# Xiaoming-Zhao/PointNav-VO

Measured on AMD Instinct MI355X. Metric: RGB-D frame-pair VO inferences/s @341x192, higher is better.
Workload: dtype f32

## Files before the change

### pointnav-vo_amd/csrc/pnvo_api.hip

```cpp
#include <hip/hip_runtime.h>

#include <cmath>
#include <cstdio>
#include <cstdlib>
#include <cstring>
#include <functional>
#include <atomic>
#include <condition_variable>
#include <map>
#include <mutex>
#include <string>
#include <thread>
#include <vector>

#include "pnvo_model.h"

using namespace pnvo;

thread_local std::string g_err;

int pnvo_fail(pnvo_handle h, int code, const std::string &msg) {
  if (h) h->err = msg;
  g_err = msg;
  return code;
}

long long pnvo_device_bytes_live(void) { return g_device_bytes_live.load(); }

namespace {

inline int fail(pnvo_handle h, int code, const std::string &msg) { return pnvo_fail(h, code, msg); }


Layer make_layer(const std::string &name, const std::string &gn, int cin, int cout, int k, int stride, int pad,
                 int hin, int win, int groups) {
  Layer l;
  l.name = name;
  l.gn = gn;
  l.cin = cin;
  l.cinp = rup(cin, 8);
  l.cout = cout;
  l.coutp = rup(cout, 32);
  l.k = l.kw = k;
  l.stride = stride;
  l.pad = pad;
  l.hin = hin;
  l.win = win;
  l.hout = (hin + 2 * pad - k) / stride + 1;
  l.wout = (win + 2 * pad - k) / stride + 1;
  l.groups = groups;
  return l;
}

void build_plan(pnvo_model_s *m) {
  const pnvo_config &c = m->cfg;
  m->C = c.n_rgb + c.n_depth + c.n_dd + c.n_tdv;
  m->CP = rup(m->C, 8);
  m->CPL = rup(m->C, 16);
  m->Hs = halve(c.height);
  m->Ws = halve(c.width);
  m->Hp = halve(m->Hs);
  m->Wp = halve(m->Ws);
  {
    const int n[4] = {c.n_rgb, c.n_depth, c.n_dd, c.n_tdv};
    int prev_off[4], half = 0;
    for (int t = 0; t < 4; ++t) {
      prev_off[t] = half;
// ... 128 lines not shown
              if (co < cout && ci < cin)
                out[((((size_t)ntg * T + tap) * J + j) * 64 + hh * 32 + n) * 4 + t] =
                    oihw[((size_t)co * cin + ci) * T + tap];
            }
}

namespace {
inline void pack_conv_weight_cinp(const float *oihw, int cout, int cin, int cinp, int kh, int kw, std::vector<float> &out) {
  pnvo_pack_conv_weight_cinp(oihw, cout, cin, cinp, kh, kw, out);
}

int load_conv(pnvo_handle h, const Toc &t, Layer &l, bool has_gn) {
  int rc = PNVO_OK;
  const float *w = find_tensor(h, t, l.name + ".weight", {l.cout, l.cin / l.cgroups, l.k, l.kw}, &rc);
  if (!w) return rc;
  if (l.cgroups > 1) {
    const int cg = l.cin / l.cgroups;
    if (l.cin != l.cout || !conv_group_supported(l.cout, cg, l.k, l.stride, l.pad))
      return fail(h, PNVO_ERR_ARG, "grouped conv " + l.name + ": unsupported geometry (" + std::to_string(l.cout) + " channels in groups of " +
                                       std::to_string(cg) + ")");
    std::vector<float> pk(conv_group_packed_floats(l.cout, cg));
    pack_conv_group_weight(w, l.cout, cg, pk.data());
    HIPCHK(h, l.wpk_grp.upload(pk.data(), pk.size()));
  } else {
    std::vector<float> pk;
    pack_conv_weight_cinp(w, l.cout, l.cin, l.cinp, l.k, l.kw, pk);
    HIPCHK(h, l.wpk.upload(pk.data(), pk.size()));
    l.host_w.assign(w, w + (size_t)l.cout * l.cin * l.k * l.kw);
  }
  if (has_gn) {
    const float *g = find_tensor(h, t, l.gn + ".weight", {l.cout}, &rc);
    if (!g) return rc;
    const float *b = find_tensor(h, t, l.gn + ".bias", {l.cout}, &rc);
    if (!b) return rc;
    HIPCHK(h, l.gamma.upload(g, l.cout));
    HIPCHK(h, l.beta.upload(b, l.cout));
  }
  return PNVO_OK;
}

int reset_contract_flag(pnvo_handle h) {
  if (!h->dd_flag) HIPCHK(h, h->dd_flag.alloc_host(1, hipHostMallocMapped | hipHostMallocCoherent));
  if (!h->dd_flag_dev) HIPCHK(h, h->dd_flag_dev.alloc(1));
  *(volatile int *)h->dd_flag = 0;
  HIPCHK(h, hipMemset(h->dd_flag_dev, 0, sizeof(int)));
  return PNVO_OK;
}

void free_workspace(pnvo_model_s *m) {
  pnvo_drop_graphs(m);
  for (DevBuf<float> *b : {&m->xin, &m->stem_raw, &m->out_ws, &m->bufY[0], &m->bufY[1], &m->rawA, &m->rawB, &m->rawD, &m->rawC, &m->comp_raw,
                           &m->hid, &m->stats, &m->stats_ds, &m->tapbuf})
    b->reset();
  for (DevPair<float> *q : {&m->ssA, &m->ssB, &m->ssD, &m->ssC, &m->ssE}) q->reset();
  m->cap = 0;
}

bool x3_layer(pnvo_handle m, const Layer &l) {
  const bool s2 = l.stride == 2 && m->opt.x3_s2;
  const bool k3 = l.k == 3 && l.kw == 3 && l.pad == 1 && (l.stride == 1 || s2);
  const bool k1 = l.k == 1 && l.kw == 1 && l.pad == 0 && s2;
  return (k3 || k1) && l.cgroups == 1 && !l.host_w.empty() && m->opt.conv <= 1;
}
bool x3_two_pieces(pnvo_handle m, const Layer &l) {
  if (m->bottleneck || !(l.in_bound < 6.0e4f)) return false;
  if (m->train != nullptr)
    return m->opt.train_pieces == 2 && pnvo_train_x2_scale(m, l.name + ".weight") != nullptr;
  return m->opt.pieces == 2;
}
void conv_geometry(const Layer &l, int B, int y_cstride, ConvArgs &a) {
  std::memset(&a, 0, sizeof(a));
  a.B = B;
  a.H = l.hin;
  a.W = l.win;
  a.CIN = l.cinp;
  a.Ho = l.hout;
  a.Wo = l.wout;
  a.COUT = l.cout;
  a.COUTP = l.coutp;
  a.KH = l.k;
  a.KW = l.kw;
  a.stride = l.stride;
  a.pad = l.pad;
  a.y_cstride = y_cstride;
  a.up = 1;
}

double conv_flops(const Layer &l, int B) { return 2.0 * ((double)((long)B * l.hout * l.wout) * l.cout * (l.cin / l.cgroups) * l.k * l.kw); }
double conv_bytes(const Layer &l, int B) {
  return 4.0 * ((double)B * l.hin * l.win * l.cin + (double)((long)B * l.hout * l.wout) * l.cout + (double)l.cout * l.cin * l.k * l.kw);
}

bool ride_fits(pnvo_handle m, const Layer &c1, const Layer &cd) {
  if (!m->opt.ds_fuse || m->tap_dst != nullptr || m->bottleneck || cd.k != 1 || cd.kw != 1 || cd.stride != 2 || cd.pad != 0) return false;
  if (c1.cinp != cd.cinp || c1.coutp != cd.coutp || c1.cout != cd.cout || c1.hout != cd.hout || c1.wout != cd.wout || c1.hin != cd.hin ||
      c1.win != cd.win || c1.cout != c1.coutp || c1.groups != cd.groups || cd.host_w.empty())
    return false;
  return x3_layer(m, cd) && x3_two_pieces(m, cd);
}
}

ConvChoice pnvo_conv_choice(pnvo_handle m, const Layer &l, int B, const ConvAsk &ask) {
  ConvChoice c;
  const int P = l.hout * l.wout;
  c.flops = conv_flops(l, B);
  if (l.cgroups > 1) {
// ... 28 lines not shown
  c.family = lds ? ConvChoice::FP32_LDS : ConvChoice::FP32_GENERIC;
  c.slots = lds ? conv3_lds_slots(a) : conv_slots(P, c.MT);
  return c;
}

bool pnvo_conv_takes_tail(pnvo_handle m, const Layer &l, int B) {
  return m->tap_dst == nullptr && m->opt.tail && pnvo_conv_choice(m, l, B, {}).family == ConvChoice::X3;
}

namespace {
size_t stats_floats(pnvo_handle m, const Layer &l, int B) {
  const PnvoOptions saved = m->opt;
  int slots = 0;
  m->opt.x3_s2 = 1;
  for (m->opt.conv = 1; m->opt.conv <= 3; ++m->opt.conv) slots = std::max(slots, pnvo_conv_choice(m, l, B, {}).slots);
  m->opt = saved;
  return (size_t)B * (size_t)slots * l.coutp * 2;
}

int stem_slots(pnvo_handle m, StemPlan::Kernel k) {
  if (k == StemPlan::GENERIC) return 0;
  if (k == StemPlan::LDS) return stem_tiles_x(m->Ws) * stem_tiles_y(m->Hs);
  return k == StemPlan::MX ? stem_mx_slots(m->Hs, m->Ws) : stem_dd_slots(m->Hs, m->Ws);
}

int ensure_workspace(pnvo_handle m, int B) {
  if (B <= m->cap) return PNVO_OK;
  free_workspace(m);
  const pnvo_config &c = m->cfg;
  const size_t npix = (size_t)B * c.height * c.width;
  size_t act = (size_t)B * m->Hp * m->Wp * c.baseplanes;
  for (size_t k = 1; k < m->convs.size(); ++k) {
    const size_t need = (size_t)B * m->convs[k].hout * m->convs[k].wout * m->convs[k].coutp;
    if (need > act) act = need;
  }
  int maxc = m->comp_cp;
  size_t st = 0;
  for (StemPlan::Kernel k : {StemPlan::MX, StemPlan::DD, StemPlan::LDS}) st = std::max(st, (size_t)B * stem_slots(m, k) * m->convs[0].coutp * 2);
  for (const Layer &l : m->convs) {
    if (l.coutp > maxc) maxc = l.coutp;
    const size_t s = stats_floats(m, l, B);
    if (s > st) st = s;
  }
  (void)npix;
  HIPCHK(m, m->stem_raw.alloc((size_t)B * m->Hs * m->Ws * c.baseplanes));
  HIPCHK(m, m->bufY[0].alloc(act));
  HIPCHK(m, m->bufY[1].alloc(act));
  HIPCHK(m, m->rawA.alloc(act));
  HIPCHK(m, m->rawB.alloc(act));
  HIPCHK(m, m->rawD.alloc(act));
  if (m->bottleneck) HIPCHK(m, m->rawC.alloc(act));
  HIPCHK(m, m->comp_raw.alloc((size_t)B * m->fh * m->fw * m->comp_cp));
  HIPCHK(m, m->hid.alloc((size_t)B * c.hidden));
  HIPCHK(m, m->out_ws.alloc((size_t)B * c.out_dim));
  HIPCHK(m, m->stats.alloc(st));
  HIPCHK(m, m->stats_ds.alloc(st));
  for (int k = 0; k < 2; ++k) {
    HIPCHK(m, m->ssA.alloc(k, (size_t)B * maxc));
    HIPCHK(m, m->ssB.alloc(k, (size_t)B * maxc));
    HIPCHK(m, m->ssD.alloc(k, (size_t)B * maxc));
    if (m->cfg.se) HIPCHK(m, m->ssE.alloc(k, (size_t)B * maxc));
    HIPCHK(m, m->ssC.alloc(k, (size_t)B * m->comp_cp));
    HIPCHK(m, hipMemset(m->ssC[k], 0, (size_t)B * m->comp_cp * sizeof(float)));
  }
  HIPCHK(m, m->tapbuf.alloc((size_t)B * m->fh * m->fw * m->comp_cp));
  HIPCHK(m, m->kpart.reserve((size_t)32 * B * (size_t)std::max(c.hidden, 32)));
  m->cap = B;
  return PNVO_OK;
}

}

PnvoTimed::PnvoTimed(pnvo_model_s *m_, hipStream_t s_, const std::string &name, double flops, double bytes) : m(m_), s(s_) {
  if (!m->timing) return;
  auto it = m->tindex.find(name);
  int idx;
  if (it == m->tindex.end()) {
    pnvo_kernel_time e;
    std::memset(&e, 0, sizeof(e));
    std::snprintf(e.name, sizeof(e.name), "%s", name.c_str());
    idx = (int)m->tentries.size();
    m->tentries.push_back(e);
    m->tindex[name] = idx;
  } else {
    idx = it->second;
  }
  m->tentries[idx].launches += 1;
  m->tentries[idx].flops += flops;
  m->tentries[idx].bytes += bytes;
  TimingRec r;
  auto get = [&]() {
    hipEvent_t e;
    if (!m->evpool.empty()) {
      e = m->evpool.back();
      m->evpool.pop_back();
    } else {
      (void)hipEventCreate(&e);
    }
    return e;
  };
  r.a = get();
  r.b = get();
  r.entry = idx;
  (void)hipEventRecord(r.a, s);
  m->trecs.push_back(r);
  rec = (int)m->trecs.size() - 1;
// ... 512 lines not shown
  GnGroup sgg{0x7fffffff, 0x7fffffff, {nullptr, nullptr}, {nullptr, nullptr}};
  switch (p.kernel) {
    case StemPlan::MX: rc = stem_launch_mx(m, B, r, p, sgg); break;
    case StemPlan::DD: rc = stem_launch_dd(m, B, r, p); break;
    case StemPlan::LDS: {
      StemArgs a;
      stem_lds_args(m, B, r, p.slots, a);
      a.dbg = m->opt.stem_dbg;
      a.lds_pad = m->opt.stem_dbg_pad;
      Timed t = stem_timed(m, B, r, false);
      HIPCHK(m, launch_stem_lds(a, stem.coutp, r.s));
      break;
    }
    case StemPlan::GENERIC:
      return pnvo_run_conv(m, stem, B, {.in_scale = m->stem_sc, .in_shift = m->stem_sh, .y = r.y, .y_cstride = stem.coutp, .ss = r.ss,
                                        .mu = r.mu, .rstd = r.rstd, .src = r.src, .grp = r.grp, .s = r.s});
  }
  if (rc != PNVO_OK) return rc;
  if (p.kernel != StemPlan::LDS) {
    if (p.repairs && (rc = pnvo_stem_standin(m, B, r, p.slots, m->dd_flag_dev)) != PNVO_OK) return rc;
    if ((rc = pnvo_mark_stem(m, r.s, p)) != PNVO_OK) return rc;
  }
  if (r.slots_out != nullptr) *r.slots_out = p.slots;
  return r.skip_finalize ? PNVO_OK : finalize_gn(m, stem, B, p.slots, 0, r.ss, r.mu, r.rstd, r.s, r.grp ? &sgg : nullptr);
}

int pnvo_ensure_workspace(pnvo_handle m, int B) { return ensure_workspace(m, B); }

namespace {
struct OptChoice {
  const char *word;
  int value;
};
struct OptDef {
  const char *key, *env;
  int PnvoOptions::*field;
  bool numeric;
  OptChoice choices[7];
};
const OptDef kOptions[] = {
    {"stem", "PNVO_STEM", &PnvoOptions::stem, false, {{"auto", 0}, {"mx", 1}, {"dd", 2}, {"dense", 3}, {nullptr, 0}}},
    {"conv", "PNVO_CONV", &PnvoOptions::conv, false, {{"auto", 0}, {"x3", 1}, {"fp32", 2}, {"generic", 3}, {nullptr, 0}}},
    {"pieces", "PNVO_PIECES", &PnvoOptions::pieces, false, {{"2", 2}, {"3", 3}, {nullptr, 0}}},
    {"stem_form", "PNVO_STEM_FORM", &PnvoOptions::stem_form, false, {{"auto", 0}, {"tiles", 2}, {"resident", 3}, {"fast", 4}, {nullptr, 0}}},
    {"train_pieces", "PNVO_TRAIN_PIECES", &PnvoOptions::train_pieces, false, {{"2", 2}, {"3", 3}, {nullptr, 0}}},
    {"x3_persist", "PNVO_X3_PERSIST", &PnvoOptions::x3_persist, false, {{"on", 1}, {"off", 0}, {nullptr, 0}}},
    {"x3_rows", "PNVO_X3_ROWS", &PnvoOptions::x3_rows, false, {{"on", 1}, {"off", 0}, {nullptr, 0}}},
    {"x3_strip", "PNVO_X3_STRIP", &PnvoOptions::x3_strip, false, {{"on", 1}, {"off", 0}, {nullptr, 0}}},
    {"x3_fine", "PNVO_X3_FINE", &PnvoOptions::x3_fine, false, {{"on", 1}, {"off", 0}, {nullptr, 0}}},
    {"x3_w8", "PNVO_X3_W8", &PnvoOptions::x3_w8, false, {{"on", 1}, {"off", 0}, {nullptr, 0}}},
    {"x3_m16", "PNVO_X3_M16", &PnvoOptions::x3_m16, false, {{"on", 1}, {"off", 0}, {nullptr, 0}}},
    {"x3_ksplit", "PNVO_X3_KSPLIT", &PnvoOptions::x3_ksplit, false, {{"on", 1}, {"off", 0}, {nullptr, 0}}},
    {"fc_rows", "PNVO_FC_ROWS", &PnvoOptions::fc_rows, true, {{nullptr, 0}}},
    {"head_fuse", "PNVO_HEAD_FUSE", &PnvoOptions::head_fuse, false, {{"on", 1}, {"off", 0}, {nullptr, 0}}},
    {"ds_fuse", "PNVO_DS_FUSE", &PnvoOptions::ds_fuse, false, {{"on", 1}, {"off", 0}, {nullptr, 0}}},
    {"gn_fuse", "PNVO_GN_FUSE", &PnvoOptions::gn_fuse, false, {{"on", 1}, {"off", 0}, {nullptr, 0}}},
    {"x3_s2", nullptr, &PnvoOptions::x3_s2, false, {{"on", 1}, {"off", 0}, {nullptr, 0}}},
    {"tail", "PNVO_TAIL", &PnvoOptions::tail, false, {{"fused", 1}, {"separate", 0}, {nullptr, 0}}},
    {"pool", "PNVO_POOL", &PnvoOptions::pool, false, {{"fused", 1}, {"separate", 0}, {nullptr, 0}}},
    {"graph", "PNVO_GRAPH", &PnvoOptions::graph, true, {{nullptr, 0}}},
    {"stem_dbg", nullptr, &PnvoOptions::stem_dbg, true, {{nullptr, 0}}},
    {"stem_dbg_pad", nullptr, &PnvoOptions::stem_dbg_pad, true, {{nullptr, 0}}},
    {"wgrad_stem", "PNVO_WGRAD_STEM", &PnvoOptions::wgrad_stem, false, {{"mx", 0}, {"fp32", 1}, {nullptr, 0}}},
    {"wgrad3", "PNVO_WGRAD3", &PnvoOptions::wgrad3, false, {{"x3", 1}, {"fp32", 0}, {nullptr, 0}}},
    {"pool_bwd", "PNVO_POOL_BWD", &PnvoOptions::pool_bwd, false, {{"fused", 1}, {"separate", 0}, {nullptr, 0}}},
    {"dgrad", "PNVO_DGRAD", &PnvoOptions::dgrad, false, {{"phase", 1}, {"masked", 0}, {nullptr, 0}}},
    {"bf16_fuse", nullptr, &PnvoOptions::bf16_fuse, false, {{"on", 1}, {"off", 0}, {nullptr, 0}}},
    {"input_fallback", "PNVO_INPUT_FALLBACK", &PnvoOptions::input_fallback, false, {{"on", 1}, {"off", 0}, {nullptr, 0}}},
    {"small_net", "PNVO_SMALL_NET", &PnvoOptions::small_net, false, {{"on", 1}, {"off", 0}, {nullptr, 0}}},
    {"small_max", "PNVO_SMALL_MAX", &PnvoOptions::small_max, true, {{nullptr, 0}}},
    {"small_coop", "PNVO_SMALL_COOP", &PnvoOptions::small_coop, true, {{nullptr, 0}}},
    {"small_prof", "PNVO_SMALL_PROF", &PnvoOptions::small_prof, true, {{nullptr, 0}}},
};

const OptDef *find_option(const char *key) {
  for (const OptDef &d : kOptions)
    if (std::strcmp(d.key, key) == 0) return &d;
  return nullptr;
}

bool parse_option(const OptDef &d, const char *word, int *out) {
  if (d.numeric) {
    char *end = nullptr;
    const long v = std::strtol(word, &end, 10);
    if (end == word || *end != 0) return false;
    *out = (int)v;
    return true;
  }
  for (const OptChoice *c = d.choices; c->word != nullptr; ++c)
    if (std::strcmp(c->word, word) == 0) {
      *out = c->value;
      return true;
    }
  return false;
}

void env_defaults(pnvo_model_s *m) {
  for (const OptDef &d : kOptions) {
    const char *e = d.env ? std::getenv(d.env) : nullptr;
    int v;
    if (e && parse_option(d, e, &v)) m->opt.*(d.field) = v;
  }
  if (std::getenv("PNVO_X3_S2_OFF")) m->opt.x3_s2 = 0;
  if (std::getenv("PNVO_BF16_NOFUSE")) m->opt.bf16_fuse = 0;
  if (const char *e = std::getenv("PNVO_STEM_DBG")) std::sscanf(e, "%d,%d", &m->opt.stem_dbg, &m->opt.stem_dbg_pad);
}
// ... 245 lines not shown
            double ind = 0.0;
            for (int k = 0; k < 30; ++k) {
              const int r = ref[k];
              if (r < 0) continue;
              const double wv = (double)w[((size_t)o * st.cin + r) * T + tap];
              const double sd = (double)h->stdev[r], mu = (double)h->mean[r];
              const double div = slot_tensor[k] == 0 ? 255.0 : 1.0;
              wk[((size_t)o * 32 + k) * T + tap] = (float)(wv / (div * sd));
              ind -= wv * mu / sd;
            }
            wk[((size_t)o * 32 + 30) * T + tap] = (float)ind;
          }
      };
      fold(slot_ref, h->mx_wk);
      fold(slot_ref_sw, h->mx_wk_swapped);
      h->mx_slot_ref = slot_ref;
      h->mx_slot_new = slot_new;
      std::vector<unsigned short> pk(stem_mx_packed_u16(3, st.cout / 32));
      pack_stem_mx_weight(h->mx_wk.data(), st.cout, 3, h->mx_xslot, pk.data());
      HIPCHK(h, h->mx_wpk3.upload(pk.data(), pk.size()));
      {
        std::vector<unsigned short> pk2(stem_mx_packed_u16(2, st.cout / 32));
        h->mx_oscale = pack_stem_mx_weight_h(h->mx_wk.data(), st.cout, h->mx_xslot, pk2.data());
        h->mx_wpk2_dev = false;
        HIPCHK(h, h->mx_wpk2.upload(pk2.data(), pk2.size()));
      }
      {
        std::vector<float> pages(64, 0.f);
        HIPCHK(h, h->mx_pages.upload(pages.data(), pages.size()));
      }
      if ((rc = reset_contract_flag(h)) != PNVO_OK) return rc;
      h->mx_ok = true;
    }
  }
  const int flat = h->comp_c * h->fh * h->fw;
  const int fc_in = flat + (c.act_embed ? 32 : 0);
  const float *w1 = find_tensor(h, t, h->fc.name + ".weight", {c.hidden, fc_in}, &rc);
  if (!w1) return rc;
  const float *b1 = find_tensor(h, t, h->fc.name + ".bias", {c.hidden}, &rc);
  if (!b1) return rc;
  {
    std::vector<float> vis((size_t)c.hidden * flat);
    for (int o = 0; o < c.hidden; ++o) std::memcpy(&vis[(size_t)o * flat], w1 + (size_t)o * fc_in, sizeof(float) * flat);
    std::vector<float> pk;
    h->fc.host_w = vis;
    {
      const int hw = h->fh * h->fw, kp = hw * h->comp_cp;
      std::vector<float> rows((size_t)c.hidden * kp, 0.f);
      for (int o = 0; o < c.hidden; ++o)
        for (int ch = 0; ch < h->comp_c; ++ch)
          for (int q = 0; q < hw; ++q) rows[(size_t)o * kp + (size_t)q * h->comp_cp + ch] = vis[(size_t)o * flat + (size_t)ch * hw + q];
      HIPCHK(h, h->fc_rows_w.upload(rows.data(), rows.size()));
    }
    pack_conv_weight_cinp(vis.data(), c.hidden, h->comp_c, h->comp_cp, h->fh, h->fw, pk);
    HIPCHK(h, h->fc.wpk.upload(pk.data(), pk.size()));
    const int rows = c.act_embed ? c.n_acts + 1 : 1;
    std::vector<float> bias((size_t)rows * c.hidden);
    const float *emb = nullptr;
    if (c.act_embed) {
      emb = find_tensor(h, t, "action_embedding.weight", {c.n_acts + 1, 32}, &rc);
      if (!emb) return rc;
    }
    for (int a = 0; a < rows; ++a)
      for (int o = 0; o < c.hidden; ++o) {
        double acc = 0.0;
        if (emb)
          for (int e = 0; e < 32; ++e) acc += (double)w1[(size_t)o * fc_in + flat + e] * (double)emb[a * 32 + e];
        bias[(size_t)a * c.hidden + o] = (float)(acc + (double)b1[o]);
      }
    HIPCHK(h, h->fc_bias.upload(bias.data(), bias.size()));
  }
  const float *w2 = find_tensor(h, t, "output_head.1.weight", {c.out_dim, c.hidden}, &rc);
  if (!w2) return rc;
  const float *b2 = find_tensor(h, t, "output_head.1.bias", {c.out_dim}, &rc);
  if (!b2) return rc;
  {
    std::vector<float> pk;
    h->head.host_w.assign(w2, w2 + (size_t)c.out_dim * c.hidden);
    pack_conv_weight_cinp(w2, c.out_dim, c.hidden, c.hidden, 1, 1, pk);
    HIPCHK(h, h->head.wpk.upload(pk.data(), pk.size()));
    HIPCHK(h, h->head_bias.upload(b2, c.out_dim));
    HIPCHK(h, h->head_w_plain.upload(w2, (size_t)c.out_dim * c.hidden));
  }
  h->loaded = true;
  h->load_gen += 1;
  h->weights_gen += 1;
  h->weights_gen_at_load = h->weights_gen;
  return PNVO_OK;
}

int pnvo_set_option(pnvo_handle h, const char *key, const char *value) {
  if (!h || !key || !value) return fail(h, PNVO_ERR_ARG, "null argument");
  const OptDef *d = find_option(key);
  if (!d) return fail(h, PNVO_ERR_ARG, std::string("unknown option '") + key + "'");
  int v;
  if (!parse_option(*d, value, &v)) {
    std::string msg = std::string("option '") + key + "' does not take '" + value + "' (";
    if (d->numeric) msg += "an integer";
    for (const OptChoice *c = d->choices; !d->numeric && c->word != nullptr; ++c) msg += std::string(c == d->choices ? "" : " | ") + c->word;
    return fail(h, PNVO_ERR_ARG, msg + ")");
  }
  const bool lift = d->field == &PnvoOptions::stem && h->dense_sticky;
  if (h->opt.*(d->field) == v && !lift) return PNVO_OK;
  h->opt.*(d->field) = v;
  pnvo_drop_graphs(h);
  if (lift) {
// ... 355 lines not shown
    }
    return PNVO_OK;
  }
  return run_fc_head(m, B, m->comp_raw, m->ssC[0], m->ssC[1], r);
}

bool fc_rows_usable(pnvo_handle m, int B, const FwdRequest &r) {
  const long kp = (long)m->fh * m->fw * m->comp_cp;
  return m->opt.fc_rows >= B && B >= 1 && m->fc_rows_w != nullptr && m->train == nullptr && m->precision == 0 && m->opt.conv == 0 &&
         m->comp_cp > 0 && 256 % m->comp_cp == 0 && kp % 4 == 0 && kp / 4 <= 64L * FC_ROWS_MAXV && m->cfg.hidden % 4 == 0 &&
         (r.features_only || m->head_w_plain != nullptr);
}

int run_fc_rows(pnvo_handle m, pnvo_handle const *grp, const int *end, int ng, int B, const float *comp_raw, const float *sc, const float *sh,
                const FwdRequest &r) {
  const pnvo_config &c = m->cfg;
  FcRowsArgs a;
  std::memset(&a, 0, sizeof(a));
  a.x = comp_raw;
  a.sc = sc;
  a.sh = sh;
  a.hid = r.features_only ? r.out : m->hid;
  a.out = r.out;
  a.actions = c.act_embed ? r.actions : nullptr;
  a.B = B;
  a.Kp = m->fh * m->fw * m->comp_cp;
  a.cp = m->comp_cp;
  a.hidden = c.hidden;
  a.out_dim = c.out_dim;
  a.ngroups = ng;
  for (int k = 0; k < ng; ++k) {
    a.end[k] = end[k];
    a.w[k] = grp[k]->fc_rows_w;
    a.bias[k] = grp[k]->fc_bias;
    a.head_w[k] = grp[k]->head_w_plain;
    a.head_b[k] = grp[k]->head_bias;
  }
  Timed t(m, r.s, "conv:" + m->fc.name, 2.0 * B * (double)a.Kp * c.hidden, 4.0 * ng * (double)a.Kp * c.hidden);
  HIPCHK(m, launch_fc_rows(a, !r.features_only, r.s));
  return PNVO_OK;
}

int run_fc_head(pnvo_handle m, int B, const float *comp_raw, const float *sc, const float *sh, const FwdRequest &r) {
  const pnvo_config &c = m->cfg;
  float *out = r.out;
  hipStream_t s = r.s;
  int rc = PNVO_OK;
  if (fc_rows_usable(m, B, r)) {
    pnvo_handle one[1] = {m};
    const int end[1] = {B};
    if ((rc = run_fc_rows(m, one, end, 1, B, comp_raw, sc, sh, r)) != PNVO_OK) return rc;
    return r.features_only ? PNVO_OK : maybe_tap(m, "hidden", m->hid, (size_t)B * c.hidden, s);
  }
  bool head_rode = false;
  const float *head_w = m->train != nullptr ? pnvo_train_weight_ptr(m, "output_head.1.weight") : m->head_w_plain;
  float *head_out = (m->opt.head_fuse && !r.features_only && c.out_dim <= 4 && head_w != nullptr) ? out : nullptr;
  if ((rc = pnvo_run_conv(m, m->fc, B, {.x = comp_raw, .in_scale = sc, .in_shift = sh, .y = m->hid, .y_cstride = c.hidden, .bias = m->fc_bias,
                                        .bias_row = c.act_embed ? r.actions : nullptr, .relu_out = 1, .head_w = head_w, .head_out = head_out,
                                        .head_rode = &head_rode, .s = s})) != PNVO_OK)
    return rc;
  if ((rc = maybe_tap(m, "hidden", m->hid, (size_t)B * c.hidden, s)) != PNVO_OK) return rc;
  if (head_rode) return PNVO_OK;
  if (r.features_only) {
    HIPCHK(m, hipMemcpyAsync(out, m->hid, (size_t)B * c.hidden * sizeof(float), hipMemcpyDeviceToDevice, s));
    return PNVO_OK;
  }
  return pnvo_run_conv(m, m->head, B, {.x = m->hid, .y = out, .y_cstride = c.out_dim, .bias = m->head_bias, .s = s});
}
}

namespace {
bool raw_direct(pnvo_handle m, const float *depth_frames) {
  const StemPlan sp = pnvo_stem_plan(m, false, {});
  if (depth_frames == nullptr || !sp.raw_stager() || m->tap_dst != nullptr) return false;
  if (m->precision == 1) return true;
  return sp.h2_from_host;
}

int raw_materialise(pnvo_handle m, const uint8_t *rgb_frames, const float *depth_frames, int B, int32_t *err_flag, hipStream_t s) {
  const pnvo_config &c = m->cfg;
  if (B > m->rawws_cap) {
    for (DevBuf<float> &q : m->rawws) q.reset();
    const size_t px = (size_t)B * c.height * c.width;
    if (c.n_rgb) HIPCHK(m, m->rawws[0].alloc(px * 6));
    HIPCHK(m, m->rawws[1].alloc(px * 2));
    if (c.n_dd) HIPCHK(m, m->rawws[2].alloc(px * (size_t)c.n_dd));
    m->rawws_cap = B;
  }
  HIPCHK(m, launch_frame_pairs(c.n_rgb ? rgb_frames : nullptr, depth_frames, B, c.height, c.width, c.n_dd / 2, m->rawws[0], m->rawws[1],
                               m->rawws[2], err_flag, s));
  return PNVO_OK;
}
}

int pnvo_forward_raw(pnvo_handle m, const uint8_t *rgb_frames, const float *depth_frames, const float *tdv, const int64_t *actions, int B,
                     float *out, int32_t *err_flag, void *stream) {
  if (!m) return fail(m, PNVO_ERR_ARG, "null handle");
  if (!m->loaded) return fail(m, PNVO_ERR_STATE, "pnvo_forward_raw before pnvo_load_weights");
  if (B <= 0 || !out) return fail(m, PNVO_ERR_ARG, "bad batch / null output");
  const pnvo_config &c = m->cfg;
  if ((c.n_rgb > 0) != (rgb_frames != nullptr) || ((c.n_depth > 0 || c.n_dd > 0) && depth_frames == nullptr) ||
      (c.n_tdv > 0) != (tdv != nullptr))
    return fail(m, PNVO_ERR_ARG, "sensor frames do not match the model's observation_space");
  if (c.act_embed && !actions) return fail(m, PNVO_ERR_ARG, "act_embed model needs actions");
  if (int rc0 = pnvo_check_inputs(m)) return rc0;
  HIPCHK(m, hipSetDevice(m->device));
// ... 490 lines not shown
```

### pointnav-vo_amd/csrc/pnvo_internal.h

```cpp
#pragma once
#include <mutex>
#include <hip/hip_runtime.h>
#include <stdint.h>

namespace pnvo {

constexpr int PNVO_ABSMAX_UINTS = 64 * 16;

struct SrcPiece {
  const float *base;
  int nch;
  int choff;
};

struct ConvArgs {
  const float *x;
  const float *wpk;
  float *y;
  const float *in_scale;
  const float *in_shift;
  float *stats;
  const float *bias;
  const int64_t *bias_row;
  int B, H, W, CIN;
// ... 198 lines not shown
hipError_t launch_conv_x2_scales(const float *params, const long *seg_dev, int nseg, float *out, hipStream_t s);
hipError_t launch_conv_x2_repack(const float *w_oihw, int cout, int cin, int cinp, int coutp, int kh, int kw, const float *scale_dev,
                                 unsigned short *out, hipStream_t s, int transposed = 0);
float pack_conv_x2_weight(const float *oihw, int cout, int cin, int cinp, int coutp, int kh, int kw, unsigned short *out);

struct ConvBArgs {
  const unsigned short *x[2];
  const unsigned short *wpk[2];
  void *y[2];
  const float *in_scale[2], *in_shift[2];
  const unsigned short *x2[2];
  const float *in_scale2[2], *in_shift2[2];
  unsigned short *xout[2];
  float *stats[2];
  int B, H, W, CIN, Ho, Wo, COUTP;
  int TR, TC, tiles_r, tiles_c, PR, PC, CK, MT, wn, slots;
  int persist_wgs;
  const unsigned short *ds_wpk[2];
  void *ds_y[2];
  float *ds_stats[2];
  const float *ds_gamma[2], *ds_beta[2];
  float *ds_scale[2], *ds_shift[2];
  const float *gn_gamma[2], *gn_beta[2];
  float *gn_scale[2], *gn_shift[2];
  int gn_cpg;
  float gn_eps;
  long gn_P;
};
bool conv_bf16_plan(ConvBArgs &a, int ks, int stride, int *mw, int *nw, size_t *lds_bytes);
hipError_t launch_conv_bf16(const ConvBArgs &a, int ks, int stride, int mode, bool f32out, int mw, int nw, size_t lds_bytes,
                            int nmodels, hipStream_t s);
void pack_conv_bf16_weight(const float *oihw, int cout, int cin, int cinp, int coutp, int kh, int kw, unsigned short *out);
hipError_t launch_gn_relu_maxpool_bf16(const unsigned short *const *x, const float *const *scale, const float *const *shift,
                                       int B, int H, int W, int C, unsigned short *const *out, int nmodels, hipStream_t s);
hipError_t launch_residual_bf16(const unsigned short *const *a, const float *const *sa, const float *const *ta,
                                const unsigned short *const *b, const float *const *sb, const float *const *tb, int B, long P,
                                int C, unsigned short *const *y, int nmodels, hipStream_t s);

int conv_slots(int P, int MT);
void choose_tile(long M, int COUTP, int *MT, int *NT);
hipError_t launch_conv(const ConvArgs &a, hipStream_t s);
hipError_t launch_ksplit_reduce(const ConvArgs &a, hipStream_t s);
constexpr int FC_ROWS_MAXV = 12;
struct FcRowsArgs {
  const float *x, *sc, *sh;
  float *hid, *out;
  const int64_t *actions;
  int B, Kp, cp, hidden, out_dim, ngroups;
  int end[3];
  const float *w[3], *bias[3], *head_w[3], *head_b[3];
};
hipError_t launch_fc_rows(const FcRowsArgs &a, bool with_head, hipStream_t s);
hipError_t launch_ksplit_reduce_head(const ConvArgs &a, const float *w2, const float *b2, int out_dim, float *out, hipStream_t s);
int conv_ksplit(const ConvArgs &a);

bool conv3_lds_supported(const ConvArgs &a);
int conv3_lds_slots(const ConvArgs &a);
hipError_t launch_conv3_lds(const ConvArgs &a, int nt, hipStream_t s);

size_t packed_conv_floats(int cout, int cin, int kh, int kw);
void pack_conv_weight(const float *oihw, int cout, int cin, int kh, int kw, float *out);

struct GnGroup {
  int end0, end1;
  const float *gamma[2], *beta[2];
};
hipError_t launch_gn_finalize(const float *stats, int B, int slots, int CP, int C, int G, long P, int WM,
                              const float *gamma, const float *beta, float eps, float *scale, float *shift,
                              hipStream_t s, int fixed_ns = 0, float *mu_out = nullptr, float *rstd_out = nullptr,
                              const GnGroup *grp = nullptr);

hipError_t launch_gn_finalize_pair(const float *const *stats, int B, int slots, int CP, int C, int G, long P, const float *const *gamma,
                                   const float *const *beta, float eps, float *const *scale, float *const *shift, float *const *mu_out,
                                   float *const *rstd_out, hipStream_t s, const GnGroup *grp0 = nullptr, const GnGroup *grp1 = nullptr);
hipError_t launch_gn_finalize2(const float *const *stats, int B, int slots, int CP, int C, int G, long P, const float *const *gamma,
                               const float *const *beta, float eps, float *const *scale, float *const *shift, int nmodels,
                               hipStream_t s);

struct AssembleArgs {
  const float *src[4];
  int nsrc[4];
  const float *mean;
  const float *stdev;
  int C, CP;
  long npix;
  float *out;
};
hipError_t launch_assemble(const AssembleArgs &a, hipStream_t s);

hipError_t launch_gn_relu_maxpool(const float *x, const float *scale, const float *shift, int B, int H, int W,
                                  int C, float *out, hipStream_t s);

hipError_t launch_flag_publish(const int *dev_flag, int *host_flag, hipStream_t s);

inline bool pnvo_first_launch_on_device(std::mutex &mu, unsigned long long &seen) {
  int dev = 0;
  if (hipGetDevice(&dev) != hipSuccess) return true;
  const unsigned long long bit = 1ull << (dev & 63);
  std::lock_guard<std::mutex> lk(mu);
  if (seen & bit) return false;
  seen |= bit;
  return true;
}

hipError_t launch_pool_keys_from_raw(const float *x, const float *gamma, int B, int H, int W, int C, int *keys, const int *only_if,
                                     hipStream_t s);
// ... 149 lines not shown
```

### pointnav-vo_amd/csrc/pnvo_model.h

```cpp
#pragma once
#include <hip/hip_runtime.h>

#include <map>
#include <functional>
#include <string>
#include <vector>

#include "../../include/pnvo.h"
#include "pnvo_internal.h"
#include "dev_buf.h"

using pnvo::DevBuf;
using pnvo::DevPair;

static inline int rup(int x, int m) { return (x + m - 1) / m * m; }
static inline int halve(int x) { return (x - 1) / 2 + 1; }

struct Layer {
  std::string name, gn;
  int cin = 0, cinp = 0, cout = 0, coutp = 0, k = 1, kw = 1, stride = 1, pad = 0;
  int hin = 0, win = 0, hout = 0, wout = 0, groups = 1;
  DevBuf<float> wpk, gamma, beta;
  std::vector<float> host_w;
  DevBuf<unsigned short> wpk_x3;
  unsigned long long x3_gen = 0;
  DevBuf<unsigned short> wpk_x2;
  unsigned long long x2_gen = 0;
  float x2_oscale = 1.f;
  float in_bound = 3.0e38f;
  int block = -1;
  int cgroups = 1;
  DevBuf<float> wpk_grp;
};

struct Block {
  int stage = 0, index = 0;
  int nconv = 0;
  int conv[3] = {-1, -1, -1};
  int ds = -1;
  std::string tap;
  int se_r = 0;
  DevBuf<float> se_w1, se_b1, se_w2, se_b2;
};

struct PnvoOptions {
  int stem = 0;
  int conv = 0;
  int stem_form = 0;
  int pieces = 2;
  int train_pieces = 2;
  int x3_rows = 1;
  int x3_persist = 1;
  int x3_strip = 1;
  int x3_fine = 1;
  int x3_m16 = 1;
  int x3_w8 = 1;
  int x3_ksplit = 1;
  int fc_rows = 48;
  int head_fuse = 1;
  int ds_fuse = 1;
  int gn_fuse = 1;
  int x3_s2 = 1;
  int tail = 1;
  int pool = 1;
  int graph = 0;
  int stem_dbg = 0, stem_dbg_pad = 0;
  int wgrad_stem = 0;
  int wgrad3 = 1;
  int pool_bwd = 1;
  int dgrad = 1;
  int bf16_fuse = 1;
  int input_fallback = 1;
  int small_net = 1;
  int small_max = 3;
  int small_prof = 0;
  int small_coop = 1;
};

struct TimingRec {
  hipEvent_t a, b;
  int entry;
};

struct pnvo_model_s {
  pnvo_config cfg;
  int device = 0;
  std::string err;
  std::string note;
  bool loaded = false;

  int C = 0, CP = 0;
  int Hs = 0, Ws = 0, Hp = 0, Wp = 0, fh = 0, fw = 0, comp_c = 0, comp_cp = 0;
  std::vector<Layer> convs;
  std::vector<Block> blocks;
  int comp = -1;
  const Layer &last(const Block &b) const { return convs[b.conv[b.nconv - 1]]; }
  int next_conv_after(size_t k) const { return k + 1 < blocks.size() ? blocks[k + 1].conv[0] : comp; }
  Layer fc, head;
  DevBuf<float> fc_bias, head_bias;
  DevBuf<float> fc_rows_w;
  DevBuf<float> head_w_plain;
  std::vector<float> mean, stdev;
  std::vector<int> stem_ref_of_new;
  std::vector<int> stem_tensor_of_new, stem_ch_of_new;
  DevBuf<float> stem_sc, stem_sh, zero_page;
  DevBuf<float> kpart;
  DevBuf<float> stem_wpk16;
  int CPL = 0;
  bool dd_ok = false;
  int dd_bins = 0;
  std::vector<int> dd_dense_tensor, dd_dense_ch;
  DevBuf<float> dd_wpk, dd_table, dd_sc, dd_sh;
  DevBuf<int> dd_flag;
  DevBuf<int> dd_flag_dev;
  DevBuf<unsigned long long> dd_prof;

  bool mx_ok = false;
  DevBuf<unsigned short> mx_wpk3;
  DevBuf<unsigned short> mx_wpk2;
  float mx_oscale = 1.f;
  DevBuf<float> mx_scale2_dev;
  bool mx_wpk2_dev = false;
  std::vector<float> mx_wk, mx_wk_swapped;
  int mx_xslot[4] = {-1, -1, -1, -1};
  std::vector<int> mx_slot_ref, mx_slot_new;
  DevBuf<float> mx_pages;
  DevBuf<unsigned long long> mx_prof;
  bool mx_prof_rs = false;
  int num_cus = 256;
  bool train_mx = false;
  PnvoOptions opt;
  bool dense_sticky = false;
  int fallback_count = 0;
  DevBuf<float> stats_ds;
  hipEvent_t stem_ev = nullptr;
  bool stem_ev_pending = false;
  DevBuf<float> rawws[3];
  int rawws_cap = 0;
  int precision = 0;
  unsigned long long load_gen = 0;
  unsigned long long weights_gen_at_load = 0;
  unsigned long long uid = 0;
  unsigned long long weights_gen = 0;
  void *bf = nullptr;

  int cap = 0;
  DevBuf<float> xin, stem_raw, bufY[2];
  DevBuf<float> rawA, rawB, rawD, rawC, comp_raw, hid, stats;
  bool bottleneck = false;
  bool grouped_se = false;
  DevPair<float> ssA, ssB, ssD, ssC;
  DevPair<float> ssE;
  DevBuf<float> tapbuf;
// ... 173 lines not shown
```

Measured before the change: 117,600.

## Add split-fp16 MFMA path for the large-batch visual FC layer

Adds a three-kernel path for the flattened visual FC layer at batches above the fc_rows threshold. The first kernel applies the GroupNorm scale/shift and ReLU, then splits the activations into fp16 hi/lo pairs. The second runs three 32x32x16 fp16 MFMAs per step (hi*hi, hi*lo, lo*hi) against pre-split, exponent-scaled weights, using buffer loads prefetched into registers and a two-way K split. The third reduces the halves, adds bias and ReLU, and optionally fuses the output head; the cost is an extra packing pass, partial-sum traffic and an approximate emulation of fp32.

Measured after the change: 118,000 (median of 3 runs). Within noise of the previous version (+0.3%).

```diff
diff --git a/pointnav-vo_amd/csrc/fc_x2.hip b/pointnav-vo_amd/csrc/fc_x2.hip
--- /dev/null
+++ b/pointnav-vo_amd/csrc/fc_x2.hip
@@ -0,0 +1,155 @@
+#include "fc_x2_pack.h"
+#include "pnvo_internal.h"
+
+namespace pnvo {
+
+typedef float f32x16 __attribute__((ext_vector_type(16)));
+typedef float f32x4 __attribute__((ext_vector_type(4)));
+typedef float f32x2 __attribute__((ext_vector_type(2)));
+typedef _Float16 f16x8 __attribute__((ext_vector_type(8)));
+typedef _Float16 f16x2 __attribute__((ext_vector_type(2)));
+typedef unsigned u32x4 __attribute__((ext_vector_type(4)));
+
+static_assert(FC_X2_STEP_PAD == 8 * FC_X2_G, "every wave walks whole groups of FC_X2_G steps");
+
+namespace {
+__device__ __forceinline__ unsigned pack2h(float a, float b) {
+  const f16x2 r = __builtin_convertvector(f32x2{a, b}, f16x2);
+  return __builtin_bit_cast(unsigned, r);
+}
+}
+
+__global__ __launch_bounds__(256) void fc_x2_split_kernel(const FcX2Args p) {
+  const int lane = threadIdx.x & 63, row = lane & 31, h = lane >> 5;
+  const int mt = blockIdx.x, s = (int)blockIdx.y * 4 + (int)(threadIdx.x >> 6);
+  const int b = mt * 32 + row, k = 16 * s + 8 * h;
+  float a[8];
+#pragma unroll
+  for (int e = 0; e < 8; ++e) a[e] = 0.f;
+  if (b < p.B && k < p.Kp) {
+    const int c = k % p.cp;
+    const float *x = p.x + (long)b * p.Kp + k, *sc = p.sc + (long)b * p.cp + c, *sh = p.sh + (long)b * p.cp + c;
+    const f32x4 v0 = *reinterpret_cast<const f32x4 *>(x), v1 = *reinterpret_cast<const f32x4 *>(x + 4);
+    const f32x4 sc0 = *reinterpret_cast<const f32x4 *>(sc), sc1 = *reinterpret_cast<const f32x4 *>(sc + 4);
+    const f32x4 sh0 = *reinterpret_cast<const f32x4 *>(sh), sh1 = *reinterpret_cast<const f32x4 *>(sh + 4);
+#pragma unroll
+    for (int e = 0; e < 4; ++e) {
+      a[e] = c + e < p.C ? fmaxf(__builtin_fmaf(v0[e], sc0[e], sh0[e]), 0.f) : 0.f;
+      a[4 + e] = c + 4 + e < p.C ? fmaxf(__builtin_fmaf(v1[e], sc1[e], sh1[e]), 0.f) : 0.f;
+    }
+  }
+  u32x4 a0, a1;
+#pragma unroll
+  for (int e = 0; e < 4; ++e) {
+    const f16x2 hh = __builtin_convertvector(f32x2{a[2 * e], a[2 * e + 1]}, f16x2);
+    a0[e] = __builtin_bit_cast(unsigned, hh);
+    a1[e] = pack2h(a[2 * e] - (float)hh[0], a[2 * e + 1] - (float)hh[1]);
+  }
+  u32x4 *dst = reinterpret_cast<u32x4 *>(p.apk) + ((long)mt * p.steps + s) * 128 + lane;
+  dst[0] = a0;
+  dst[64] = a1;
+}
+
+__global__ __launch_bounds__(256) void fc_x2_kernel(const FcX2Args p) {
+  __shared__ float part[4 * 16 * 64];
+  const int lane = threadIdx.x & 63;
+  const int wave = __builtin_amdgcn_readfirstlane(threadIdx.x >> 6);
+  const int MT = (p.B + 31) >> 5, NT = p.hidden >> 5, nitems = 2 * MT * NT;
+  const int chunk = (nitems + 7) >> 3;
+  const int t = (int)(blockIdx.x & 7) * chunk + (int)(blockIdx.x >> 3);
+  if (t >= nitems) return;
+  const int z = t & 1, mt = (t >> 1) % MT, nt = (t >> 1) / MT;
+  const int n = p.steps >> 3;
+  const __amdgpu_buffer_rsrc_t ra = __builtin_amdgcn_make_buffer_rsrc((void *)p.apk, 0, MT * p.steps * 2048, 0x00020000);
+  const __amdgpu_buffer_rsrc_t rw = __builtin_amdgcn_make_buffer_rsrc((void *)p.wpk, 0, NT * p.steps * 2048, 0x00020000);
+  const int abase = (mt * p.steps + (4 * z + wave) * n) * 2048 + lane * 16, wbase = (nt * p.steps + (4 * z + wave) * n) * 2048 + lane * 16;
+
+  f32x16 acc;
+#pragma unroll
+  for (int r = 0; r < 16; ++r) acc[r] = 0.f;
+  u32x4 a0[FC_X2_G], a1[FC_X2_G], w0[FC_X2_G], w1[FC_X2_G];
+  auto fetch = [&](int u, int s) {
+    a0[u] = __builtin_bit_cast(u32x4, __builtin_amdgcn_raw_buffer_load_b128(ra, abase + s * 2048, 0, 0));
+    a1[u] = __builtin_bit_cast(u32x4, __builtin_amdgcn_raw_buffer_load_b128(ra, abase + s * 2048 + 1024, 0, 0));
+    w0[u] = __builtin_bit_cast(u32x4, __builtin_amdgcn_raw_buffer_load_b128(rw, wbase + s * 2048, 0, 0));
+    w1[u] = __builtin_bit_cast(u32x4, __builtin_amdgcn_raw_buffer_load_b128(rw, wbase + s * 2048 + 1024, 0, 0));
+  };
+#pragma unroll
+  for (int u = 0; u < FC_X2_G; ++u) {
+    fetch(u, u);
+    __builtin_amdgcn_sched_barrier(0);
+  }
+  for (int s = 0; s < n; s += FC_X2_G) {
+#pragma unroll
+    for (int u = 0; u < FC_X2_G; ++u) {
+      acc = __builtin_amdgcn_mfma_f32_32x32x16_f16(__builtin_bit_cast(f16x8, a1[u]), __builtin_bit_cast(f16x8, w0[u]), acc, 0, 0, 0);
+      acc = __builtin_amdgcn_mfma_f32_32x32x16_f16(__builtin_bit_cast(f16x8, a0[u]), __builtin_bit_cast(f16x8, w1[u]), acc, 0, 0, 0);
+      acc = __builtin_amdgcn_mfma_f32_32x32x16_f16(__builtin_bit_cast(f16x8, a0[u]), __builtin_bit_cast(f16x8, w0[u]), acc, 0, 0, 0);
+      fetch(u, min(s + u + FC_X2_G, n - 1));
+      __builtin_amdgcn_sched_barrier(0);
+    }
+  }
+
+#pragma unroll
+  for (int r = 0; r < 16; ++r) part[(wave * 16 + r) * 64 + lane] = acc[r];
+  __syncthreads();
+  const int h = lane >> 5, col = nt * 32 + (lane & 31);
+  float *dst = p.part + (long)z * p.B * p.hidden;
+#pragma unroll
+  for (int i = 0; i < 4; ++i) {
+    const int r = 4 * wave + i;
+    const float v = ((part[(0 * 16 + r) * 64 + lane] + part[(1 * 16 + r) * 64 + lane]) + part[(2 * 16 + r) * 64 + lane]) + part[(3 * 16 + r) * 64 + lane];
+    const int b = mt * 32 + 8 * wave + 4 * h + i;
+    if (b < p.B) dst[(long)b * p.hidden + col] = v * p.oscale;
+  }
+}
+
+__global__ __launch_bounds__(256) void fc_x2_head_kernel(const float *part, long M, int C, const float *bias, const int64_t *bias_row, float *hid,
+                                                       const float *w2, const float *b2, int OD, float *out) {
+  __shared__ float red[4][4];
+  const long m = blockIdx.x;
+  const float *brow = bias + (bias_row != nullptr ? (long)bias_row[m] : 0) * C;
+  float acc[4] = {0.f, 0.f, 0.f, 0.f};
+  for (int c = (int)threadIdx.x; c < C; c += 256) {
+    const float v = fmaxf((part[m * C + c] + part[(M + m) * C + c]) + brow[c], 0.f);
+    hid[m * C + c] = v;
+#pragma unroll
+    for (int o = 0; o < 4; ++o)
+      if (o < OD) acc[o] = __builtin_fmaf(v, w2[(long)o * C + c], acc[o]);
+  }
+  if (OD <= 0) return;
+#pragma unroll
+  for (int o = 0; o < 4; ++o)
+#pragma unroll
+    for (int d = 32; d >= 1; d >>= 1) acc[o] += __shfl_xor(acc[o], d);
+  const int wave = (int)(threadIdx.x >> 6);
+  if ((threadIdx.x & 63) == 0)
+#pragma unroll
+    for (int o = 0; o < 4; ++o) red[wave][o] = acc[o];
+  __syncthreads();
+  if ((int)threadIdx.x < OD) {
+    const int o = (int)threadIdx.x;
+    out[m * OD + o] = (((red[0][o] + red[1][o]) + red[2][o]) + red[3][o]) + b2[o];
+  }
+}
+
+bool fc_x2_supported(int B, int Kp, int cp, int hidden) {
+  return B >= 1 && hidden >= 32 && hidden % 32 == 0 && cp >= 8 && cp % 8 == 0 && Kp >= cp && Kp % cp == 0;
+}
+
+size_t fc_x2_act_u16(int B, int Kp) { return (size_t)((B + 31) / 32) * fc_x2_steps(Kp) * 2 * 64 * 8; }
+
+hipError_t launch_fc_x2(const FcX2Args &a, const float *head_w, const float *head_b, int out_dim, float *out, hipStream_t s) {
+  if (!fc_x2_supported(a.B, a.Kp, a.cp, a.hidden) || a.steps != fc_x2_steps(a.Kp) || a.C > a.cp || a.apk == nullptr || a.part == nullptr ||
+      (head_w != nullptr && (out_dim < 1 || out_dim > 4)))
+    return hipErrorInvalidValue;
+  const int MT = (a.B + 31) / 32, nitems = 2 * MT * (a.hidden / 32);
+  const int chunk = (nitems + 7) / 8;
+  hipLaunchKernelGGL(fc_x2_split_kernel, dim3((unsigned)MT, (unsigned)(a.steps / 4)), dim3(256), 0, s, a);
+  hipLaunchKernelGGL(fc_x2_kernel, dim3((unsigned)(8 * chunk)), dim3(256), 0, s, a);
+  hipLaunchKernelGGL(fc_x2_head_kernel, dim3((unsigned)a.B), dim3(256), 0, s, a.part, (long)a.B, a.hidden, a.bias, a.bias_row, a.hid, head_w,
+                     head_b, head_w != nullptr ? out_dim : 0, out);
+  return hipGetLastError();
+}
+
+}
diff --git a/pointnav-vo_amd/csrc/fc_x2_pack.h b/pointnav-vo_amd/csrc/fc_x2_pack.h
--- /dev/null
+++ b/pointnav-vo_amd/csrc/fc_x2_pack.h
@@ -0,0 +1,47 @@
+#pragma once
+#include <cmath>
+#include <cstddef>
+#include <cstring>
+
+namespace pnvo {
+
+constexpr int FC_X2_G = 9;
+constexpr int FC_X2_STEP_PAD = 8 * FC_X2_G;
+inline int fc_x2_steps(int Kp) { return ((Kp + 15) / 16 + FC_X2_STEP_PAD - 1) / FC_X2_STEP_PAD * FC_X2_STEP_PAD; }
+inline size_t fc_x2_packed_u16(int hidden, int Kp) { return (size_t)(hidden / 32) * fc_x2_steps(Kp) * 2 * 64 * 8; }
+
+inline float pack_fc_x2_weight(const float *w, int hidden, int C, int cp, int hw, unsigned short *out) {
+  const int flat = C * hw, Kp = hw * cp, steps = fc_x2_steps(Kp), ntt = hidden / 32;
+  float mx = 0.f;
+  for (size_t k = 0; k < (size_t)hidden * flat; ++k) mx = std::fmax(mx, std::fabs(w[k]));
+  int e = 0;
+  if (mx > 0.f) std::frexp(mx, &e);
+  const float scale = std::ldexp(1.0f, 12 - e), inv = std::ldexp(1.0f, e - 12);
+  auto to_h = [](float f) {
+    const _Float16 h = (_Float16)f;
+    unsigned short u;
+    std::memcpy(&u, &h, 2);
+    return u;
+  };
+  auto to_f = [](unsigned short u) {
+    _Float16 h;
+    std::memcpy(&h, &u, 2);
+    return (float)h;
+  };
+  for (int nt = 0; nt < ntt; ++nt)
+    for (int s = 0; s < steps; ++s)
+      for (int ln = 0; ln < 64; ++ln)
+        for (int j = 0; j < 8; ++j) {
+          const int o = nt * 32 + (ln & 31), k = 16 * s + 8 * (ln >> 5) + j;
+          const int q = k / cp, ch = k - q * cp;
+          float v = 0.f;
+          if (k < Kp && ch < C) v = w[(size_t)o * flat + (size_t)ch * hw + q] * scale;
+          const unsigned short h0 = to_h(v);
+          const size_t base = (((size_t)nt * steps + s) * 2) * 512 + (size_t)ln * 8 + j;
+          out[base] = h0;
+          out[base + 512] = to_h(v - to_f(h0));
+        }
+  return inv;
+}
+
+}
diff --git a/pointnav-vo_amd/csrc/pnvo_api.hip b/pointnav-vo_amd/csrc/pnvo_api.hip
--- a/pointnav-vo_amd/csrc/pnvo_api.hip
+++ b/pointnav-vo_amd/csrc/pnvo_api.hip
@@ -13,6 +13,7 @@
 #include <thread>
 #include <vector>
 
+#include "fc_x2_pack.h"
 #include "pnvo_model.h"
 
 using namespace pnvo;
@@ -247,6 +248,7 @@
   for (DevBuf<float> *b : {&m->xin, &m->stem_raw, &m->out_ws, &m->bufY[0], &m->bufY[1], &m->rawA, &m->rawB, &m->rawD, &m->rawC, &m->comp_raw,
                            &m->hid, &m->stats, &m->stats_ds, &m->tapbuf})
     b->reset();
+  m->fc_x2_a.reset();
   for (DevPair<float> *q : {&m->ssA, &m->ssB, &m->ssD, &m->ssC, &m->ssE}) q->reset();
   m->cap = 0;
 }
@@ -381,6 +383,7 @@
   if (m->bottleneck) HIPCHK(m, m->rawC.alloc(act));
   HIPCHK(m, m->comp_raw.alloc((size_t)B * m->fh * m->fw * m->comp_cp));
   HIPCHK(m, m->hid.alloc((size_t)B * c.hidden));
+  if (m->fc_x2_w != nullptr) HIPCHK(m, m->fc_x2_a.alloc(fc_x2_act_u16(B, m->fh * m->fw * m->comp_cp)));
   HIPCHK(m, m->out_ws.alloc((size_t)B * c.out_dim));
   HIPCHK(m, m->stats.alloc(st));
   HIPCHK(m, m->stats_ds.alloc(st));
@@ -999,6 +1002,7 @@
     {"x3_m16", "PNVO_X3_M16", &PnvoOptions::x3_m16, false, {{"on", 1}, {"off", 0}, {nullptr, 0}}},
     {"x3_ksplit", "PNVO_X3_KSPLIT", &PnvoOptions::x3_ksplit, false, {{"on", 1}, {"off", 0}, {nullptr, 0}}},
     {"fc_rows", "PNVO_FC_ROWS", &PnvoOptions::fc_rows, true, {{nullptr, 0}}},
+    {"fc_x2", "PNVO_FC_X2", &PnvoOptions::fc_x2, false, {{"on", 1}, {"off", 0}, {nullptr, 0}}},
     {"head_fuse", "PNVO_HEAD_FUSE", &PnvoOptions::head_fuse, false, {{"on", 1}, {"off", 0}, {nullptr, 0}}},
     {"ds_fuse", "PNVO_DS_FUSE", &PnvoOptions::ds_fuse, false, {{"on", 1}, {"off", 0}, {nullptr, 0}}},
     {"gn_fuse", "PNVO_GN_FUSE", &PnvoOptions::gn_fuse, false, {{"on", 1}, {"off", 0}, {nullptr, 0}}},
@@ -1350,6 +1354,13 @@
           for (int q = 0; q < hw; ++q) rows[(size_t)o * kp + (size_t)q * h->comp_cp + ch] = vis[(size_t)o * flat + (size_t)ch * hw + q];
       HIPCHK(h, h->fc_rows_w.upload(rows.data(), rows.size()));
     }
+    if (fc_x2_supported(1, h->fh * h->fw * h->comp_cp, h->comp_cp, c.hidden)) {
+      std::vector<unsigned short> pk2(fc_x2_packed_u16(c.hidden, h->fh * h->fw * h->comp_cp));
+      h->fc_x2_oscale = pack_fc_x2_weight(vis.data(), c.hidden, h->comp_c, h->comp_cp, h->fh * h->fw, pk2.data());
+      HIPCHK(h, h->fc_x2_w.upload(pk2.data(), pk2.size()));
+    } else {
+      h->fc_x2_w.reset();
+    }
     pack_conv_weight_cinp(vis.data(), c.hidden, h->comp_c, h->comp_cp, h->fh, h->fw, pk);
     HIPCHK(h, h->fc.wpk.upload(pk.data(), pk.size()));
     const int rows = c.act_embed ? c.n_acts + 1 : 1;
@@ -1811,6 +1822,33 @@
     if ((rc = run_fc_rows(m, one, end, 1, B, comp_raw, sc, sh, r)) != PNVO_OK) return rc;
     return r.features_only ? PNVO_OK : maybe_tap(m, "hidden", m->hid, (size_t)B * c.hidden, s);
   }
+  if (m->opt.fc_x2 && B > m->opt.fc_rows && m->fc_x2_w != nullptr && m->train == nullptr && m->precision == 0 && m->opt.conv <= 1 && m->opt.pieces == 2 &&
+      fc_x2_supported(B, m->fh * m->fw * m->comp_cp, m->comp_cp, c.hidden)) {
+    const int Kp = m->fh * m->fw * m->comp_cp;
+    const bool head_here = m->opt.head_fuse && !r.features_only && c.out_dim <= 4 && m->head_w_plain != nullptr;
+    if (fc_x2_act_u16(B, Kp) > m->fc_x2_a.size()) {
+      pnvo_drop_graphs(m);
+      HIPCHK(m, m->fc_x2_a.alloc(fc_x2_act_u16(B, Kp)));
+    }
+    if ((size_t)2 * B * c.hidden > m->kpart.size()) {
+      pnvo_drop_graphs(m);
+      HIPCHK(m, m->kpart.alloc((size_t)2 * B * c.hidden));
+    }
+    {
+      Timed t(m, s, "conv:" + m->fc.name, conv_flops(m->fc, B), conv_bytes(m->fc, B));
+      HIPCHK(m, launch_fc_x2({.x = comp_raw, .sc = sc, .sh = sh, .wpk = m->fc_x2_w, .apk = m->fc_x2_a, .bias = m->fc_bias,
+                              .bias_row = c.act_embed ? r.actions : nullptr, .part = m->kpart, .hid = m->hid, .oscale = m->fc_x2_oscale, .B = B,
+                              .Kp = Kp, .cp = m->comp_cp, .C = m->comp_c, .hidden = c.hidden, .steps = fc_x2_steps(Kp)},
+                             head_here ? (const float *)m->head_w_plain : nullptr, m->head_bias, c.out_dim, out, s));
+    }
+    if ((rc = maybe_tap(m, "hidden", m->hid, (size_t)B * c.hidden, s)) != PNVO_OK) return rc;
+    if (head_here) return PNVO_OK;
+    if (r.features_only) {
+      HIPCHK(m, hipMemcpyAsync(out, m->hid, (size_t)B * c.hidden * sizeof(float), hipMemcpyDeviceToDevice, s));
+      return PNVO_OK;
+    }
+    return pnvo_run_conv(m, m->head, B, {.x = m->hid, .y = out, .y_cstride = c.out_dim, .bias = m->head_bias, .s = s});
+  }
   bool head_rode = false;
   const float *head_w = m->train != nullptr ? pnvo_train_weight_ptr(m, "output_head.1.weight") : m->head_w_plain;
   float *head_out = (m->opt.head_fuse && !r.features_only && c.out_dim <= 4 && head_w != nullptr) ? out : nullptr;
diff --git a/pointnav-vo_amd/csrc/pnvo_internal.h b/pointnav-vo_amd/csrc/pnvo_internal.h
--- a/pointnav-vo_amd/csrc/pnvo_internal.h
+++ b/pointnav-vo_amd/csrc/pnvo_internal.h
@@ -274,6 +274,20 @@
 };
 hipError_t launch_fc_rows(const FcRowsArgs &a, bool with_head, hipStream_t s);
 hipError_t launch_ksplit_reduce_head(const ConvArgs &a, const float *w2, const float *b2, int out_dim, float *out, hipStream_t s);
+struct FcX2Args {
+  const float *x, *sc, *sh;
+  const unsigned short *wpk;
+  unsigned short *apk;
+  const float *bias;
+  const int64_t *bias_row;
+  float *part;
+  float *hid;
+  float oscale;
+  int B, Kp, cp, C, hidden, steps;
+};
+bool fc_x2_supported(int B, int Kp, int cp, int hidden);
+size_t fc_x2_act_u16(int B, int Kp);
+hipError_t launch_fc_x2(const FcX2Args &a, const float *head_w, const float *head_b, int out_dim, float *out, hipStream_t s);
 int conv_ksplit(const ConvArgs &a);
 
 bool conv3_lds_supported(const ConvArgs &a);
diff --git a/pointnav-vo_amd/csrc/pnvo_model.h b/pointnav-vo_amd/csrc/pnvo_model.h
--- a/pointnav-vo_amd/csrc/pnvo_model.h
+++ b/pointnav-vo_amd/csrc/pnvo_model.h
@@ -57,6 +57,7 @@
   int x3_w8 = 1;
   int x3_ksplit = 1;
   int fc_rows = 48;
+  int fc_x2 = 1;
   int head_fuse = 1;
   int ds_fuse = 1;
   int gn_fuse = 1;
@@ -99,6 +100,9 @@
   Layer fc, head;
   DevBuf<float> fc_bias, head_bias;
   DevBuf<float> fc_rows_w;
+  DevBuf<unsigned short> fc_x2_w;
+  float fc_x2_oscale = 1.f;
+  DevBuf<unsigned short> fc_x2_a;
   DevBuf<float> head_w_plain;
   std::vector<float> mean, stdev;
   std::vector<int> stem_ref_of_new;
```
